# rapidsai/cugraph-gnn

Hardware: AMD Instinct MI355X
Metric: sampled-edges/sec (sample+renumber+feature-gather+SAGEConv fwd), ogbn-products-like fan-out [25, 10] (higher is better)
Workload: dtype int64 ids (int32 timed as a variant) + f32 features (SAGE lin_l/lin_r product: bf16x3-split MFMA, f32 accumulate); 1 GPU; ogbn-products-like RMAT: V=2449029, E=118462496 directed (CSR row_ptr i64 / col i64 replicated per GPU), feat fp32 [V,100], batch 1024/GPU, fan-out [25, 10], 2-layer SAGEConv(mean) 100-256-47 fwd, step = 8 call groups of 188 mini-batches; parallelism=dp1 (seeds sharded, no data-path collective)

## Files before the change

cugraph-gnn_amd/csrc/wg_rng.hpp:

```cpp
#pragma once
#include <hip/hip_runtime.h>

#include <cstdint>

namespace wgamd {

struct PcgJump {
  uint64_t a;
  uint64_t s;
};

struct PcgJumpTables {
  PcgJump t[4][256];
  constexpr PcgJumpTables() : t{}
  {
    uint64_t base_a = 6364136223846793005ULL, base_s = 1;
    for (int k = 0; k < 4; k++) {
      t[k][0].a = 1;
      t[k][0].s = 0;
      for (int c = 1; c < 256; c++) {
        t[k][c].a = t[k][c - 1].a * base_a;
        t[k][c].s = t[k][c - 1].s * base_a + base_s;
      }
      for (int d = 0; d < 8; d++) {
        uint64_t na = base_a * base_a, ns = base_s * base_a + base_s;
        base_a = na;
        base_s = ns;
      }
    }
  }
};

__device__ __constant__ const PcgJumpTables g_pcg_jump{};

struct Pcg32 {
  uint64_t state;
  uint64_t inc;

  static constexpr uint64_t kMult = 6364136223846793005ULL;

  __host__ __device__ __forceinline__ uint32_t next_u32()
  {
    uint64_t old = state;
    state        = old * kMult + inc;
    uint32_t x   = (uint32_t)(((old >> 18u) ^ old) >> 27u);
    uint32_t rot = (uint32_t)(old >> 59u);
    return (x >> rot) | (x << ((0u - rot) & 31u));
  }

  __host__ __device__ __forceinline__ void skipahead(uint64_t delta)
  {
    uint64_t acc_mult = 1u, acc_plus = 0u, cur_mult = kMult, cur_plus = inc;
    while (delta) {
      if (delta & 1u) {
        acc_mult *= cur_mult;
        acc_plus = acc_plus * cur_mult + cur_plus;
      }
      cur_plus = (cur_mult + 1u) * cur_plus;
      cur_mult *= cur_mult;
      delta >>= 1u;
    }
    state = acc_mult * state + acc_plus;
  }

  __host__ __device__ __forceinline__ Pcg32(uint64_t seed, uint64_t subsequence)
  {
    state = 0u;
    inc   = (subsequence << 1u) | 1u;
    (void)next_u32();
    state += seed;
    (void)next_u32();
    skipahead(subsequence);
  }

  __device__ __forceinline__ void jump_table(uint32_t n)
  {
    PcgJump j = g_pcg_jump.t[0][n & 255u];
#pragma unroll
    for (int k = 1; k < 4; k++) {
      const uint32_t c = (n >> (8 * k)) & 255u;
      if (c) {
        const PcgJump m = g_pcg_jump.t[k][c];
        j.s             = j.s * m.a + m.s;
        j.a             = j.a * m.a;
      }
    }
    state = j.a * state + inc * j.s;
  }

  struct table_tag {};
  __device__ __forceinline__ Pcg32(uint64_t seed, uint32_t subsequence, table_tag, uint32_t extra_draws = 0)
  {
    inc   = ((uint64_t)subsequence << 1u) | 1u;
    state = (inc + seed) * kMult + inc;
    jump_table(subsequence + extra_draws);
  }

  __host__ __device__ __forceinline__ int32_t next_i31() { return (int32_t)(next_u32() & 0x7fffffffu); }
  __host__ __device__ __forceinline__ uint64_t next_u64()
  {
    uint64_t lo = next_u32();
    uint64_t hi = next_u32();
    return lo | (hi << 32u);
  }
  __host__ __device__ __forceinline__ int64_t next_i63() { return (int64_t)(next_u64() & 0x7fffffffffffffffULL); }
  __host__ __device__ __forceinline__ float next_f32() { return (float)(next_u32() >> 8u) / 16777216.0f; }
};

}
```

cugraph-gnn_amd/csrc/wg_sample.hip:

```cpp
#include <algorithm>
#include <cmath>

#include "wg_common.hpp"
#include "wg_rng.hpp"

namespace wgamd {
namespace {

template <typename T>
struct dtype_of;
template <>
struct dtype_of<int32_t> {
  static constexpr wholememory_dtype_t value = WHOLEMEMORY_DT_INT;
};
template <>
struct dtype_of<int64_t> {
  static constexpr wholememory_dtype_t value = WHOLEMEMORY_DT_INT64;
};

__host__ __device__ constexpr int ref_block_threads(int M)
{
  int f = (M - 1) / 32;
  return f < 3 ? 32 : f < 6 ? 64 : f < 12 ? 128 : 256;
}
// ... 48 lines not shown
        deg = (M > 0 && deg > M) ? M : deg;
      }
      cnt[i] = deg;
      if (big_deg) big_deg[i] = 0;
    }
    return;
  }
  int i = blockIdx.x * blockDim.x + threadIdx.x;
  int cls          = -1;
  int deg          = 0;
  if (i < n_.host) {
    if (i >= n_live) {
      if (i < (n_live / kScanTile + 1) * kScanTile) {
        cnt[i] = 0;
        if (big_deg) big_deg[i] = 0;
      }
    } else {
      int64_t nid         = (int64_t)seeds[i];
      const int64_t first = row_ptr[nid];
      deg                 = (int)(row_ptr[nid + 1] - first);
      cnt[i]              = (M > 0 && deg > M) ? M : deg;
      if (row_start) {
        row_start[i] = first;
        row_deg[i]   = deg;
      }
      if (big_deg) big_deg[i] = 0;
      if (lists != nullptr && M > 0 && deg > M) {
        cls = deg <= 16 ? 0 : deg <= 32 ? 1 : deg <= 64 ? 2 : deg <= 128 ? 3 : deg <= 256 ? 4 : deg <= 512 ? 5
              : deg <= kWaveRowCapDecl ? 6 : deg <= kHugeRow ? 7 : 8;
        if (cls >= 7 && deg > scratch_threshold) atomicMax(lists + 10, deg);
      }
    }
  }
  if (lists == nullptr) return;
  __shared__ int blk_cnt[kWeightedLists], blk_base[kWeightedLists];
  if (threadIdx.x < kWeightedLists) blk_cnt[threadIdx.x] = 0;
  __syncthreads();
  const int lane = threadIdx.x & 63;
  int my_rank    = 0;
#pragma unroll
  for (int c = 0; c < kWeightedLists; c++) {
    const uint64_t m = __ballot(cls == c);
    if (m == 0ull) continue;
    const int leader = __ffsll((long long)m) - 1;
    int base         = 0;
    if (lane == leader) base = atomicAdd(&blk_cnt[c], __popcll(m));
    base = __shfl(base, leader, 64);
    if (cls == c) my_rank = base + __popcll(m & ((1ull << lane) - 1ull));
  }
  __syncthreads();
  if (threadIdx.x < kWeightedLists && blk_cnt[threadIdx.x] > 0) blk_base[threadIdx.x] = atomicAdd(lists + threadIdx.x, blk_cnt[threadIdx.x]);
  __syncthreads();
  if (cls >= 0) lists[kWeightedListHead + (int64_t)cls * list_cap + blk_base[cls] + my_rank] = i;
}

template <typename ColT>
__device__ __forceinline__ ColT col_at(const ColT* __restrict__ col, int64_t at)
{
  return col ? col[at] : (ColT)0;
}

constexpr int kWalkGrid = 256 * 16;

template <typename ColT>
__device__ __forceinline__ void emit(ColT* dst, int* src_lid, int64_t* edge_gid, int64_t out, ColT v,
                                     int seed_index, int64_t gid)
{
  if (dst) dst[out] = v;
  if (src_lid) src_lid[out] = seed_index;
  if (edge_gid) edge_gid[out] = gid;
}

struct loc_rec {
  int64_t start;
  int i;
  int deg;
  int base;
  int i_local;
  int batch;
  int pad;
};
static_assert(sizeof(loc_rec) == 32, "one 32-byte sector per record");
constexpr int kLocBuckets = 4096;
constexpr int kLocBlocks  = 128;
constexpr int kLocThreads = 1024;

template <typename SeedT>
__global__ void __launch_bounds__(kLocThreads)
locality_hist_kernel(const SeedT* __restrict__ seeds, dev_count n_, int shift, int* __restrict__ hist )
{
  __shared__ int h[kLocBuckets];
  const int n = n_.get(), per = (n + kLocBlocks - 1) / kLocBlocks;
  const int lo = min(n, (int)blockIdx.x * per), hi = min(n, lo + per);
  for (int k = threadIdx.x; k < kLocBuckets; k += kLocThreads) h[k] = 0;
  __syncthreads();
  for (int i = lo + threadIdx.x; i < hi; i += kLocThreads)
    atomicAdd(&h[min((int)((uint64_t)seeds[i] >> shift), kLocBuckets - 1)], 1);
  __syncthreads();
  for (int k = threadIdx.x; k < kLocBuckets; k += kLocThreads) hist[(int64_t)blockIdx.x * kLocBuckets + k] = h[k];
}

template <typename SeedT>
__global__ void __launch_bounds__(kLocThreads)
locality_scatter_kernel(const SeedT* __restrict__ seeds, dev_count n_, int shift, const int* __restrict__ hist,
                        const int64_t* __restrict__ row_start, const int* __restrict__ row_deg, const int* __restrict__ offsets,
                        rng_plan rng, loc_rec* __restrict__ recs)
{
  __shared__ int cursor[kLocBuckets];
  __shared__ int wave_tot[kLocThreads / 64];
  static_assert(kLocBuckets == 4 * kLocThreads, "thread t owns buckets 4 t .. 4 t + 3");
  const int n = n_.get(), per = (n + kLocBlocks - 1) / kLocBlocks;
  const int lo = min(n, (int)blockIdx.x * per), hi = min(n, lo + per);
  int tot[4] = {0, 0, 0, 0}, before[4] = {0, 0, 0, 0};
  const int4* h4 = reinterpret_cast<const int4*>(hist);
  for (int b = 0; b < kLocBlocks; b++) {
    const int4 v = h4[(int64_t)b * (kLocBuckets / 4) + threadIdx.x];
    tot[0] += v.x; tot[1] += v.y; tot[2] += v.z; tot[3] += v.w;
    if (b < (int)blockIdx.x) { before[0] += v.x; before[1] += v.y; before[2] += v.z; before[3] += v.w; }
  }
  const int sum = tot[0] + tot[1] + tot[2] + tot[3];
  int inc = sum;
  const int lane = threadIdx.x & 63, wave = threadIdx.x >> 6;
#pragma unroll
  for (int d = 1; d < 64; d <<= 1) {
    const int up = __shfl_up(inc, d, 64);
    if (lane >= d) inc += up;
  }
  if (lane == 63) wave_tot[wave] = inc;
  __syncthreads();
  int run = inc - sum;
  for (int w = 0; w < wave; w++) run += wave_tot[w];
#pragma unroll
  for (int k = 0; k < 4; k++) {
    cursor[4 * threadIdx.x + k] = run + before[k];
    run += tot[k];
  }
  __syncthreads();
  for (int i = lo + threadIdx.x; i < hi; i += kLocThreads) {
    const int j = atomicAdd(&cursor[min((int)((uint64_t)seeds[i] >> shift), kLocBuckets - 1)], 1);
    loc_rec r;
    r.start = row_start[i];
    r.i     = i;
    r.deg   = row_deg[i];
    r.base  = offsets[i];
    r.i_local = i;
    r.batch   = 0;
    if (rng.target_batch) {
      r.batch   = rng.target_batch[i];
      r.i_local = i - rng.target_seg[r.batch];
    }
    r.pad   = 0;
    recs[j] = r;
  }
}

template <typename SeedT, typename ColT, int LANES>
__global__ void __launch_bounds__(256) sample_uniform_halfwave_kernel(const int64_t* __restrict__ row_ptr,
                                                                      const ColT* __restrict__ col,
                                                                      const SeedT* __restrict__ seeds,
                                                                      dev_count n_,
                                                                      int M,
                                                                      rng_plan rng,
                                                                      const int* __restrict__ offsets,
                                                                      ColT* __restrict__ dst,
                                                                      int* __restrict__ src_lid,
                                                                      int64_t* __restrict__ edge_gid,
                                                                      const int64_t* __restrict__ row_start,
                                                                      const int* __restrict__ row_deg,
                                                                      const loc_rec* __restrict__ recs = nullptr)
{
  const int n    = n_.get();
  const int lane = threadIdx.x & 63;
  const int hl   = lane & (LANES - 1);
  const int hb   = lane & ~(LANES - 1);
  int i          = (int)(((int64_t)blockIdx.x * blockDim.x + threadIdx.x) / LANES);
  loc_rec rec{};
  if (recs) {
    constexpr int kGroups = 256 / LANES;
    const int per_x = ((n + 7) / 8 + kGroups - 1) / kGroups * kGroups;
    const int k     = (int)(blockIdx.x >> 3) * kGroups + (int)threadIdx.x / LANES;
    const int j     = (int)(blockIdx.x & 7) * per_x + k;
    i               = n;
    if (k < per_x && j < n) {
      rec = recs[j];
      i   = rec.i;
    }
  }
  int32_t r_draw = 0;
  if (i < n && hl < M) {
    uint64_t random_seed;
    int i_local;
    if (recs) {
      i_local     = rec.i_local;
      random_seed = rng.seeds_dev ? rng.seeds_dev[rec.batch] : rng.seed;
    } else
      rng.resolve(i, random_seed, i_local);
    if (i_local < (1 << 26)) {
      Pcg32 g(random_seed, (uint32_t)(i_local * 32 + hl), Pcg32::table_tag{});
      r_draw = g.next_i31();
    } else {
      Pcg32 g(random_seed, stream_id(i_local, 32, hl));
      r_draw = g.next_i31();
    }
  }
  int64_t start = 0;
  int N = 0, base = 0;
  if (i < n && recs) {
    start = rec.start;
    N     = rec.deg;
    base  = rec.base;
  } else if (i < n) {
    if (row_start) {
      start = row_start[i];
      N     = row_deg[i];
    } else {
      int64_t nid = (int64_t)seeds[i];
      start       = row_ptr[nid];
      N           = (int)(row_ptr[nid + 1] - start);
    }
    base = offsets[i];
  }
  const bool pick = N > M;
  if (__ballot(pick) == 0ull) {
    if (hl < N) emit<ColT>(dst, src_lid, edge_gid, (int64_t)base + hl, col_at<ColT>(col, start + hl), i, start + hl);
    return;
  }
  int r = 0;
  if (pick && hl < M) r = r_draw % (N - hl);
  const int tail = N - hl - 1;
  int p1 = -1, p2 = -1;
  for (int s = 0; s + 1 < M; s++) {
    const int rs    = __shfl(r, hb | s, 64);
    const bool prev = s < hl;
    p1 = (prev && rs == r) ? s : p1;
    p2 = (prev && rs == tail) ? s : p2;
  }
  int root = p2 >= 0 ? p2 : hl;
#pragma unroll
  for (int round = 0; round < (LANES == 32 ? 5 : 4); round++) root = __shfl(root, hb | root, 64);
  const int val = N - root - 1;
  const int vp1 = __shfl(val, hb | (p1 & (LANES - 1)), 64);
  const int a   = p1 >= 0 ? vp1 : r;
  if (pick) {
    if (hl < M) emit<ColT>(dst, src_lid, edge_gid, (int64_t)base + hl, col_at<ColT>(col, start + a), i, start + a);
  } else if (hl < N) {
    emit<ColT>(dst, src_lid, edge_gid, (int64_t)base + hl, col_at<ColT>(col, start + hl), i, start + hl);
  }
}

template <typename SeedT, typename ColT, int GW, int K, bool EXACT>
__global__ void __launch_bounds__(256)
sample_uniform_multi_kernel(const ColT* __restrict__ col, dev_count n_, int M_rt, rng_plan rng, const int* __restrict__ offsets,
                            ColT* __restrict__ dst, int* __restrict__ src_lid, int64_t* __restrict__ edge_gid,
                            const int64_t* __restrict__ row_start, const int* __restrict__ row_deg,
                            const loc_rec* __restrict__ recs)
{
  constexpr int kGPW    = 64 / GW;
  constexpr int kGroups = 4 * kGPW;
  constexpr int kRounds = GW <= 2 ? 1 : GW <= 4 ? 2 : GW <= 8 ? 3 : GW <= 16 ? 4 : 5;
  const int M    = EXACT ? GW : M_rt;
  const int n    = n_.get();
  const int lane = threadIdx.x & 63;
  const int grp  = lane / GW;
  const int hl   = lane - grp * GW;
  const int hb   = grp * GW;
  const bool live_group = grp < kGPW;
  const int wg_group    = (int)(threadIdx.x >> 6) * kGPW + grp;
  const int per_x = ((n + 7) / 8 + kGroups * K - 1) / (kGroups * K) * (kGroups * K);
  const int64_t n_chunks = recs ? (int64_t)(per_x / (kGroups * K)) * 8 : ((int64_t)n + kGroups * K - 1) / (kGroups * K);
  for (int64_t chunk = blockIdx.x; chunk < n_chunks; chunk += gridDim.x) {
  int i[K], N[K], base[K], i_local[K], batch[K];
  int64_t start[K];
  if (recs) {
    const int k0    = ((int)(chunk >> 3) * kGroups + wg_group) * K;
#pragma unroll
    for (int k = 0; k < K; k++) {
      const int j = (int)(chunk & 7) * per_x + k0 + k;
      i[k] = n, N[k] = 0, base[k] = 0, start[k] = 0, i_local[k] = 0, batch[k] = 0;
      if (live_group && k0 + k < per_x && j < n) {
        const loc_rec r = recs[j];
        i[k] = r.i, N[k] = r.deg, base[k] = r.base, start[k] = r.start, i_local[k] = r.i_local, batch[k] = r.batch;
      }
    }
  } else {
    const int64_t g = chunk * kGroups + wg_group;
#pragma unroll
    for (int k = 0; k < K; k++) {
      i[k] = live_group ? (int)min(g * K + k, (int64_t)n) : n;
      N[k] = 0, base[k] = 0, start[k] = 0, i_local[k] = i[k], batch[k] = 0;
      if (i[k] < n) {
        start[k] = row_start[i[k]];
        N[k]     = row_deg[i[k]];
        base[k]  = offsets[i[k]];
        if (rng.target_batch) batch[k] = rng.target_batch[i[k]];
      }
    }
    if (rng.target_batch) {
#pragma unroll
      for (int k = 0; k < K; k++)
        if (i[k] < n) i_local[k] = i[k] - rng.target_seg[batch[k]];
    }
  }
  int32_t r_draw[K];
#pragma unroll
  for (int k = 0; k < K; k++) {
    r_draw[k] = 0;
    if (i[k] < n && hl < M) {
      const uint64_t random_seed = rng.seeds_dev ? rng.seeds_dev[rng.target_batch ? batch[k] : 0] : rng.seed;
      if (i_local[k] < (1 << 26)) {
        Pcg32 g(random_seed, (uint32_t)(i_local[k] * 32 + hl), Pcg32::table_tag{});
        r_draw[k] = g.next_i31();
      } else {
        Pcg32 g(random_seed, stream_id(i_local[k], 32, hl));
        r_draw[k] = g.next_i31();
      }
    }
  }
  int a[K];
#pragma unroll
  for (int k = 0; k < K; k++) {
    const bool pick = N[k] > M;
    a[k]            = hl;
    if (__ballot(pick) != 0ull) {
      int r = 0;
      if (pick && hl < M) r = r_draw[k] % (N[k] - hl);
      const int tail = N[k] - hl - 1;
      int p1 = -1, p2 = -1;
      auto step = [&](int s) {
        const int rs    = __shfl(r, hb + s, 64);
        const bool prev = s < hl;
        p1 = (prev && rs == r) ? s : p1;
        p2 = (prev && rs == tail) ? s : p2;
      };
      if constexpr (EXACT) {
#pragma unroll
        for (int s = 0; s + 1 < GW; s++) step(s);
      } else {
        for (int s = 0; s + 1 < M; s++) step(s);
      }
      int root = p2 >= 0 ? p2 : hl;
#pragma unroll
      for (int round = 0; round < kRounds; round++) root = __shfl(root, hb + root, 64);
      const int val = N[k] - root - 1;
      const int vp1 = __shfl(val, hb + max(p1, 0), 64);
      if (pick) a[k] = p1 >= 0 ? vp1 : r;
    }
  }
  ColT v[K];
  bool on[K];
#pragma unroll
  for (int k = 0; k < K; k++) {
    on[k] = live_group && hl < (N[k] > M ? M : N[k]);
    v[k]  = on[k] ? col_at<ColT>(col, start[k] + a[k]) : (ColT)0;
  }
#pragma unroll
  for (int k = 0; k < K; k++)
    if (on[k]) emit<ColT>(dst, src_lid, edge_gid, (int64_t)base[k] + hl, v[k], i[k], start[k] + a[k]);
  }
}

constexpr int kHashSlots = 4096;

__device__ __forceinline__ int lds_hash_find(const int* keys, int pos)
{
  uint32_t h = ((uint32_t)pos * 2654435761u) & (kHashSlots - 1);
  while (true) {
    int k = keys[h];
    if (k == pos || k == -1) return (int)h;
    h = (h + 1) & (kHashSlots - 1);
  }
}

template <typename SeedT, typename ColT>
__global__ void __launch_bounds__(256) sample_uniform_block_kernel(const int64_t* __restrict__ row_ptr,
                                                                   const ColT* __restrict__ col,
                                                                   const SeedT* __restrict__ seeds,
                                                                   dev_count n_,
                                                                   int M,
                                                                   int B,
                                                                   int items,
                                                                   rng_plan rng,
                                                                   const int* __restrict__ offsets,
                                                                   ColT* __restrict__ dst,
                                                                   int* __restrict__ src_lid,
                                                                   int64_t* __restrict__ edge_gid)
{
  __shared__ int r[1024];
  __shared__ int a[1024];
  __shared__ int hkeys[kHashSlots];
  __shared__ int hvals[kHashSlots];
  const int i = blockIdx.x;
  if (i >= n_.get()) return;
  const int64_t nid   = (int64_t)seeds[i];
  const int64_t start = row_ptr[nid];
  const int N         = (int)(row_ptr[nid + 1] - start);
  if (N <= 0) return;
  const int base = offsets[i];
  if (N <= M) {
    for (int j = threadIdx.x; j < N; j += blockDim.x)
      emit<ColT>(dst, src_lid, edge_gid, (int64_t)base + j, col_at<ColT>(col, start + j), i, start + j);
    return;
  }
  for (int h = threadIdx.x; h < kHashSlots; h += blockDim.x) hkeys[h] = -1;
  if ((int)threadIdx.x < B) {
    uint64_t random_seed;
    int i_local;
    rng.resolve(i, random_seed, i_local);
    Pcg32 g(random_seed, stream_id(i_local, B, threadIdx.x));
    for (int k = 0; k < items; k++) {
      int id = k * B + threadIdx.x;
      int v  = g.next_i31();
      if (id < M) r[id] = v % (N - id);
    }
  }
  __syncthreads();
  if (threadIdx.x == 0) {
    for (int t = 0; t < M; t++) {
      const int rt = r[t], tail = N - t - 1;
      int s1     = lds_hash_find(hkeys, rt);
      int q_rt   = hkeys[s1] == rt ? hvals[s1] : rt;
      int s2     = lds_hash_find(hkeys, tail);
      int q_tail = hkeys[s2] == tail ? hvals[s2] : tail;
      a[t]       = q_rt;
      hkeys[s1]  = rt;
      hvals[s1]  = q_tail;
    }
  }
  __syncthreads();
  for (int t = threadIdx.x; t < M; t += blockDim.x)
    emit<ColT>(dst, src_lid, edge_gid, (int64_t)base + t, col_at<ColT>(col, start + a[t]), i, start + a[t]);
}

template <typename SeedT, typename ColT>
__global__ void __launch_bounds__(64) sample_uniform_reservoir_kernel(const int64_t* __restrict__ row_ptr,
                                                                      const ColT* __restrict__ col,
                                                                      const SeedT* __restrict__ seeds,
                                                                      dev_count n_,
                                                                      int M,
                                                                      rng_plan rng,
                                                                      const int* __restrict__ offsets,
                                                                      ColT* __restrict__ dst,
                                                                      int* __restrict__ src_lid,
                                                                      int64_t* __restrict__ edge_gid)
{
  const int i = blockIdx.x;
  if (i >= n_.get()) return;
  const int64_t nid   = (int64_t)seeds[i];
  const int64_t start = row_ptr[nid];
  const int N         = (int)(row_ptr[nid + 1] - start);
  if (N <= 0) return;
  const int64_t base = offsets[i];
  if (N <= M) {
    for (int j = threadIdx.x; j < N; j += blockDim.x)
      emit<ColT>(dst, src_lid, edge_gid, base + j, col_at<ColT>(col, start + j), i, start + j);
    return;
  }
  for (int s = threadIdx.x; s < M; s += blockDim.x) dst[base + s] = (ColT)s;
  __syncthreads();
  if (threadIdx.x < 32) {
    uint64_t random_seed;
    int i_local;
    rng.resolve(i, random_seed, i_local);
    Pcg32 g(random_seed, stream_id(i_local, 32, threadIdx.x));
    for (int idx = M + threadIdx.x; idx < N; idx += 32) {
      int rn = g.next_i31() % (idx + 1);
      if (rn < M) {
        if constexpr (sizeof(ColT) == 8)
          atomicMax(reinterpret_cast<long long*>(dst + base + rn), (long long)idx);
        else
          atomicMax(reinterpret_cast<int*>(dst + base + rn), idx);
      }
    }
  }
  __syncthreads();
  for (int s = threadIdx.x; s < M; s += blockDim.x) {
    int sel = (int)__hip_atomic_load(dst + base + s, __ATOMIC_RELAXED, __HIP_MEMORY_SCOPE_AGENT);
    emit<ColT>(dst, src_lid, edge_gid, base + s, col_at<ColT>(col, start + sel), i, start + sel);
  }
}

__device__ __forceinline__ float ares_key(float w, Pcg32& g, bool* redrawn = nullptr)
{
  float u = g.next_f32();
  u       = (float)(-(0.5 + 0.5 * (double)u));
  uint64_t x;
  int zero_draws = -1;
  do {
    x = g.next_u64();
    zero_draws++;
  } while (!x);
  if (redrawn != nullptr && zero_draws > 0) *redrawn = true;
  int one_bit = __clzll((long long)x) + zero_draws * 64;
  u *= exp2f((float)(-one_bit));
#ifdef WG_TUNE_CHEAP_KEY
  return u * 1.442695f * __builtin_amdgcn_rcpf(w);
#endif
  return (log1pf(u) / logf(2.0f)) * (1.0f / w);
}

constexpr int kWaveRowCap = 1024;
static_assert(kWaveRowCap == kWaveRowCapDecl, "keep the two in step");

__device__ __forceinline__ uint32_t key_bits(float k)
{
  uint32_t b = __float_as_uint(k);
  return (b & 0x80000000u) ? ~b : (b | 0x80000000u);
}

constexpr int kLdsKeys = kWeightedLdsKeys;

template <typename SeedT, typename ColT, typename WeightT, int B, int T>
__global__ void __launch_bounds__(T) sample_weighted_kernel(const int64_t* __restrict__ row_ptr,
                                                            const ColT* __restrict__ col,
                                                            const WeightT* __restrict__ weight,
                                                            const SeedT* __restrict__ seeds,
                                                            dev_count n_,
                                                            int M,
                                                            rng_plan rng,
                                                            const int* __restrict__ offsets,
                                                            uint32_t* __restrict__ slab,
                                                            int64_t slab_len,
                                                            ColT* __restrict__ dst,
                                                            int* __restrict__ src_lid,
                                                            int64_t* __restrict__ edge_gid,
                                                            int* __restrict__ lists ,
                                                            int list_cap,
                                                            int redo = 0 )
{
  static_assert(T % B == 0 && T % 64 == 0, "threads must be a multiple of the stream layout and of the wave");
  __shared__ uint32_t lds_keys[kLdsKeys];
  __shared__ int hist[256];
  __shared__ int sh_digit, sh_need, sh_redo;
  __shared__ int wave_cnt[2][T / 64];
  __shared__ int sh_li;
  const int n_live  = n_.get();
  const int n_huge  = lists && !redo ? lists[8] : 0;
  const int count   = lists ? (redo ? lists[kWeightedRedoCount] : n_huge + lists[7]) : n_live;
  uint32_t* gkeys   = slab + (int64_t)blockIdx.x * slab_len;
  int li            = blockIdx.x;
  while (true) {
  __syncthreads();
  if (lists) {
    if (threadIdx.x == 0) sh_li = atomicAdd(lists + (redo ? kWeightedRedoHead : 9), 1);
    __syncthreads();
    li = sh_li;
  }
  if (li >= count) break;
  const int i = lists ? (redo ? lists[kWeightedListHead + (int64_t)kWeightedRedoList * list_cap + li]
                         : li < n_huge ? lists[kWeightedListHead + 8 * (int64_t)list_cap + li]
                                       : lists[kWeightedListHead + 7 * (int64_t)list_cap + (li - n_huge)])
                      : li;
  if (!lists) li += gridDim.x;
  if (i >= n_live) continue;
  uint64_t random_seed;
  int i_rng;
  rng.resolve(i, random_seed, i_rng);
  const int64_t nid   = (int64_t)seeds[i];
  const int64_t start = row_ptr[nid];
  const int N         = (int)(row_ptr[nid + 1] - start);
  if (N <= 0) continue;
  const int64_t base = offsets[i];
  if (M <= 0 || N <= M) {
    for (int j = threadIdx.x; j < N; j += T)
      emit<ColT>(dst, src_lid, edge_gid, base + j, col_at<ColT>(col, start + j), i, start + j);
    continue;
  }
  const bool in_lds = N <= kLdsKeys;
  auto put = [&](int id, uint32_t k) { if (in_lds) lds_keys[id] = k; else gkeys[id] = k; };
  auto get = [&](int id) -> uint32_t {
    return in_lds ? lds_keys[id] : __hip_atomic_load(gkeys + id, __ATOMIC_RELAXED, __HIP_MEMORY_SCOPE_AGENT);
  };
  if (threadIdx.x == 0) sh_redo = 0;
  __syncthreads();
  {
    constexpr int hop = T / B;
    const int lane = threadIdx.x % B, part = threadIdx.x / B;
    const int L     = lane < N ? (N - lane + B - 1) / B : 0;
    const int share = (L + hop - 1) / hop;
    const int m0 = part * share, m1 = min(L, m0 + share);
    bool redrawn = false;
    if (m0 < m1) {
      const int64_t sid = (int64_t)i_rng * B + lane;
      Pcg32 g = (sid < (1ll << 31)) ? Pcg32(random_seed, (uint32_t)sid, Pcg32::table_tag{}, 3u * (uint32_t)m0)
                                    : Pcg32(random_seed, stream_id(i_rng, B, lane));
      if (sid >= (1ll << 31)) g.skipahead(3u * (uint64_t)m0);
      for (int m = m0; m < m1; m++) {
        const int id = lane + m * B;
        put(id, key_bits(ares_key((float)weight[start + id], g, &redrawn)));
      }
    }
    if (redrawn) sh_redo = 1;
  }
  __syncthreads();
  if (T > B && sh_redo) {
    if (threadIdx.x < B) {
      Pcg32 g = stream_generator(random_seed, i_rng, B, threadIdx.x);
      for (int id = threadIdx.x; id < N; id += B) put(id, key_bits(ares_key((float)weight[start + id], g)));
    }
    __syncthreads();
  }
  uint32_t prefix = 0, prefix_mask = 0;
  int need = M;
  for (int shift = 24; shift >= 0; shift -= 8) {
    for (int h = threadIdx.x; h < 256; h += T) hist[h] = 0;
    __syncthreads();
    for (int id = threadIdx.x; id < N; id += T) {
      uint32_t k = get(id);
      if ((k & prefix_mask) == prefix) atomicAdd(&hist[(k >> shift) & 255], 1);
    }
    __syncthreads();
    if (threadIdx.x < 64) {
      const int l  = threadIdx.x;
      const int h0 = hist[4 * l], h1 = hist[4 * l + 1], h2 = hist[4 * l + 2], h3 = hist[4 * l + 3];
// ... 1252 lines not shown
```

cugraph-gnn_amd/csrc/wg_unique.hip:

```cpp
#include "wg_common.hpp"
#include "wgamd_ext.h"

namespace wgamd {
namespace {

template <typename IdT>
__global__ void __launch_bounds__(256) unique_mark_kernel(const IdT* __restrict__ ids, int64_t n, int64_t bound, uint8_t* __restrict__ flags,
                                                          int* __restrict__ bad, const int* __restrict__ n_live)
{
  if (n_live) n = min(n, (int64_t)*n_live);
  const int64_t T = (int64_t)gridDim.x * blockDim.x;
  for (int64_t i = (int64_t)blockIdx.x * blockDim.x + threadIdx.x; i < n; i += 4 * T) {
    int64_t id[4];
    uint8_t f[4];
#pragma unroll
    for (int k = 0; k < 4; k++) id[k] = i + k * T < n ? (int64_t)ids[i + k * T] : -1;
#pragma unroll
    for (int k = 0; k < 4; k++) {
      if (id[k] >= bound) {
        *bad  = 1;
        id[k] = -1;
      }
      f[k] = id[k] >= 0 ? flags[id[k]] : 1;
    }
#pragma unroll
    for (int k = 0; k < 4; k++)
      if (f[k] == 0) flags[id[k]] = 1;
  }
}

__global__ void __launch_bounds__(256) unique_pack_kernel(const uint8_t* __restrict__ flags, int64_t n_words, uint2* __restrict__ rank,
                                                          int* __restrict__ cnt, int64_t cnt_padded)
{
  const int64_t w = (int64_t)blockIdx.x * blockDim.x + threadIdx.x;
  if (w < n_words) {
    const uint4* p = reinterpret_cast<const uint4*>(flags + w * 32);
    const uint4 a = p[0], b = p[1];
    const uint32_t v[8] = {a.x, a.y, a.z, a.w, b.x, b.y, b.z, b.w};
    uint32_t word = 0;
#pragma unroll
    for (int k = 0; k < 8; k++) {
      const uint32_t x = v[k];
      word |= ((x & 1u) | ((x >> 7) & 2u) | ((x >> 14) & 4u) | ((x >> 21) & 8u)) << (4 * k);
    }
    rank[w].x = word;
    cnt[w]    = __popc(word);
  } else if (w < cnt_padded) {
    cnt[w] = 0;
  }
}

__global__ void __launch_bounds__(256) unique_compact_kernel(uint2* __restrict__ rank, const int* __restrict__ prefix, int64_t n_words,
                                                             int64_t* __restrict__ distinct, int* __restrict__ n_distinct)
{
  const int64_t w = (int64_t)blockIdx.x * blockDim.x + threadIdx.x;
  if (w == 0 && n_distinct) *n_distinct = prefix[n_words];
  if (w >= n_words) return;
  uint32_t word = rank[w].x;
  int at        = prefix[w];
  rank[w].y     = (uint32_t)at;
  while (word) {
    const int k    = __ffs(word) - 1;
    distinct[at++] = w * 32 + k;
    word &= word - 1;
  }
}

template <typename IdT>
__global__ void __launch_bounds__(256) unique_inverse_kernel(const IdT* __restrict__ ids, int64_t n, int64_t bound, const uint2* __restrict__ rank,
                                                             int* __restrict__ inverse,
                                                             const int* __restrict__ n_live)
{
  if (n_live) n = min(n, (int64_t)*n_live);
  const int64_t T = (int64_t)gridDim.x * blockDim.x;
  for (int64_t i = (int64_t)blockIdx.x * blockDim.x + threadIdx.x; i < n; i += 4 * T) {
    int64_t id[4];
    uint2 r[4];
#pragma unroll
    for (int k = 0; k < 4; k++) id[k] = i + k * T < n ? (int64_t)ids[i + k * T] : -1;
#pragma unroll
    for (int k = 0; k < 4; k++) {
      const bool ok = id[k] >= 0 && id[k] < bound;
      r[k]          = ok ? rank[id[k] >> 5] : make_uint2(0u, 0xffffffffu);
    }
#pragma unroll
    for (int k = 0; k < 4; k++)
      if (i + k * T < n) inverse[i + k * T] = (int)r[k].y + __popc(r[k].x & ((1u << (id[k] & 31)) - 1u));
  }
}

struct unique_plan {
  size_t flags, bits, cnt, tmp, bad, total;
  int64_t n_words, cnt_padded;
};
unique_plan plan_unique(int64_t bound)
{
  unique_plan p{};
  size_t at = 0;
  auto add  = [&](size_t bytes) {
    const size_t o = at;
    at += (bytes + 255) / 256 * 256;
    return o;
  };
  p.n_words    = (bound + 31) / 32;
  p.cnt_padded = (p.n_words + kScanTile) / kScanTile * kScanTile;
  p.flags = add((size_t)p.n_words * 32);
  p.bits  = add(sizeof(uint2) * (size_t)p.n_words);
  p.cnt   = add(sizeof(int) * (size_t)(p.cnt_padded + 1));
  p.tmp   = add(sizeof(int) * (size_t)scan_tmp_ints(p.n_words));
  p.bad   = add(sizeof(int));
  p.total = at;
  return p;
}

}
}

extern "C" {

size_t wgamd_unique_bounded_workspace_bytes(int64_t id_bound)
{
  if (id_bound <= 0 || id_bound >= ((int64_t)1 << 31) - 4096) return 0;
  return wgamd::plan_unique(id_bound).total;
}

wholememory_error_code_t wgamd_unique_bounded(const void* ids, wholememory_dtype_t id_dtype, int64_t n, int64_t id_bound,
                                              int64_t* distinct, int* inverse, int* n_distinct_dev, int* out_of_bound_dev,
                                              void* workspace, size_t workspace_bytes, void* stream)
{
  return wgamd_unique_bounded_live(ids, id_dtype, n, nullptr, id_bound, distinct, inverse, n_distinct_dev, out_of_bound_dev,
                                   workspace, workspace_bytes, stream);
}

wholememory_error_code_t wgamd_unique_bounded_live(const void* ids, wholememory_dtype_t id_dtype, int64_t n, const int* n_live_dev,
                                                   int64_t id_bound, int64_t* distinct, int* inverse, int* n_distinct_dev,
                                                   int* out_of_bound_dev, void* workspace, size_t workspace_bytes, void* stream)
{
  using namespace wgamd;
  return guarded("wgamd_unique_bounded", [&] {
    WG_REQUIRE_INPUT(id_dtype == WHOLEMEMORY_DT_INT || id_dtype == WHOLEMEMORY_DT_INT64, "id dtype must be INT|INT64");
    WG_REQUIRE_INPUT(n >= 0 && n < ((int64_t)1 << 31), "bad id count");
    WG_REQUIRE_INPUT(id_bound > 0 && id_bound < ((int64_t)1 << 31) - 4096, "id_bound must be in (0, 2^31)");
    WG_REQUIRE_INPUT(n_distinct_dev && workspace && (n == 0 || (ids && distinct && inverse)), "null pointer");
    const unique_plan p = plan_unique(id_bound);
    WG_REQUIRE_INPUT(workspace_bytes >= p.total, "workspace too small: need %zu bytes", p.total);
    WG_REQUIRE_INPUT((reinterpret_cast<uintptr_t>(workspace) & 255) == 0, "workspace must be 256-byte aligned");
    hipStream_t st = static_cast<hipStream_t>(stream);
    char* base     = static_cast<char*>(workspace);
    uint8_t* flags = reinterpret_cast<uint8_t*>(base + p.flags);
    uint2* rank    = reinterpret_cast<uint2*>(base + p.bits);
    int* cnt       = reinterpret_cast<int*>(base + p.cnt);
    int* tmp       = reinterpret_cast<int*>(base + p.tmp);
    int* bad       = reinterpret_cast<int*>(base + p.bad);
    WG_HIP_CHECK(hipMemsetAsync(flags, 0, (size_t)p.n_words * 32, st));
    WG_HIP_CHECK(hipMemsetAsync(bad, 0, sizeof(int), st));
    if (n > 0) {
      const int grid = (int)std::min<int64_t>(ceil_div(n, 256), 256 * 32);
      if (id_dtype == WHOLEMEMORY_DT_INT) unique_mark_kernel<int32_t><<<grid, 256, 0, st>>>(static_cast<const int32_t*>(ids), n, id_bound, flags, bad, n_live_dev);
      else unique_mark_kernel<int64_t><<<grid, 256, 0, st>>>(static_cast<const int64_t*>(ids), n, id_bound, flags, bad, n_live_dev);
      WG_HIP_CHECK(hipGetLastError());
    }
    unique_pack_kernel<<<(int)ceil_div(p.cnt_padded, 256), 256, 0, st>>>(flags, p.n_words, rank, cnt, p.cnt_padded);
    exclusive_scan_i32(cnt, cnt, p.n_words, tmp, st);
    unique_compact_kernel<<<(int)ceil_div(p.n_words, 256), 256, 0, st>>>(rank, cnt, p.n_words, distinct, n_distinct_dev);
    WG_HIP_CHECK(hipGetLastError());
    if (n > 0) {
      const int grid = (int)std::min<int64_t>(ceil_div(n, 256), 256 * 32);
      if (id_dtype == WHOLEMEMORY_DT_INT) unique_inverse_kernel<int32_t><<<grid, 256, 0, st>>>(static_cast<const int32_t*>(ids), n, id_bound, rank, inverse, n_live_dev);
      else unique_inverse_kernel<int64_t><<<grid, 256, 0, st>>>(static_cast<const int64_t*>(ids), n, id_bound, rank, inverse, n_live_dev);
      WG_HIP_CHECK(hipGetLastError());
    }
    if (out_of_bound_dev) WG_HIP_CHECK(hipMemcpyAsync(out_of_bound_dev, bad, sizeof(int), hipMemcpyDeviceToDevice, st));
  });
}

}
```

Measured before the change: 5.377 billion sampled-edges/s.

## Replicate unique flag planes, fuse scan into pack/compact, and reuse PCG jump maps

The unique path now spreads mark writes over up to eight replicated flag planes when a plane fits in about 3 MB, so concurrent blocks contend less on the same flag bytes. The pack kernel ORs the planes together and writes per-tile popcount sums. A compact kernel does the block scan with a carry, replacing the separate global scan, memsets and D2D copy with fewer launches. Separately, the sampler reuses the previous PCG jump map when consecutive rows are adjacent, composing one table step instead of four lookups. The costs are extra plane memory and clear bandwidth, plus a serial per-tile carry loop in compact.

```diff
diff --git a/cugraph-gnn_amd/csrc/wg_rng.hpp b/cugraph-gnn_amd/csrc/wg_rng.hpp
--- a/cugraph-gnn_amd/csrc/wg_rng.hpp
+++ b/cugraph-gnn_amd/csrc/wg_rng.hpp
@@ -73,27 +73,32 @@
     skipahead(subsequence);
   }
 
-  __device__ __forceinline__ void jump_table(uint32_t n)
+  __host__ __device__ __forceinline__ static PcgJump compose(const PcgJump& n, const PcgJump& m) { return PcgJump{n.a * m.a, n.s * m.a + m.s}; }
+
+  __device__ __forceinline__ static PcgJump jump_map(uint32_t n)
   {
     PcgJump j = g_pcg_jump.t[0][n & 255u];
 #pragma unroll
     for (int k = 1; k < 4; k++) {
       const uint32_t c = (n >> (8 * k)) & 255u;
-      if (c) {
-        const PcgJump m = g_pcg_jump.t[k][c];
-        j.s             = j.s * m.a + m.s;
-        j.a             = j.a * m.a;
-      }
+      if (c) j = compose(j, g_pcg_jump.t[k][c]);
     }
-    state = j.a * state + inc * j.s;
+    return j;
+  }
+
+  __host__ __device__ __forceinline__ void jump(const PcgJump& j) { state = j.a * state + inc * j.s; }
+
+  __device__ __forceinline__ Pcg32(uint64_t seed, uint32_t subsequence, const PcgJump& j)
+  {
+    inc   = ((uint64_t)subsequence << 1u) | 1u;
+    state = (inc + seed) * kMult + inc;
+    jump(j);
   }
 
   struct table_tag {};
   __device__ __forceinline__ Pcg32(uint64_t seed, uint32_t subsequence, table_tag, uint32_t extra_draws = 0)
+      : Pcg32(seed, subsequence, jump_map(subsequence + extra_draws))
   {
-    inc   = ((uint64_t)subsequence << 1u) | 1u;
-    state = (inc + seed) * kMult + inc;
-    jump_table(subsequence + extra_draws);
   }
 
   __host__ __device__ __forceinline__ int32_t next_i31() { return (int32_t)(next_u32() & 0x7fffffffu); }
diff --git a/cugraph-gnn_amd/csrc/wg_sample.hip b/cugraph-gnn_amd/csrc/wg_sample.hip
--- a/cugraph-gnn_amd/csrc/wg_sample.hip
+++ b/cugraph-gnn_amd/csrc/wg_sample.hip
@@ -374,13 +374,19 @@
     }
   }
   int32_t r_draw[K];
+  PcgJump jmap{};
+  int jmap_of = -2;
 #pragma unroll
   for (int k = 0; k < K; k++) {
     r_draw[k] = 0;
     if (i[k] < n && hl < M) {
       const uint64_t random_seed = rng.seeds_dev ? rng.seeds_dev[rng.target_batch ? batch[k] : 0] : rng.seed;
       if (i_local[k] < (1 << 26)) {
-        Pcg32 g(random_seed, (uint32_t)(i_local[k] * 32 + hl), Pcg32::table_tag{});
+        const uint32_t sid = (uint32_t)(i_local[k] * 32 + hl);
+        if (i_local[k] == jmap_of + 1) jmap = Pcg32::compose(jmap, g_pcg_jump.t[0][32]);
+        else jmap = Pcg32::jump_map(sid);
+        jmap_of = i_local[k];
+        Pcg32 g(random_seed, sid, jmap);
         r_draw[k] = g.next_i31();
       } else {
         Pcg32 g(random_seed, stream_id(i_local[k], 32, hl));
diff --git a/cugraph-gnn_amd/csrc/wg_unique.hip b/cugraph-gnn_amd/csrc/wg_unique.hip
--- a/cugraph-gnn_amd/csrc/wg_unique.hip
+++ b/cugraph-gnn_amd/csrc/wg_unique.hip
@@ -4,11 +4,24 @@
 namespace wgamd {
 namespace {
 
+constexpr int kMaxPlanes = 8;
+constexpr int64_t kPlaneL2Bytes = (int64_t)3 << 20;
+constexpr int kTileWords = 256;
+
+__global__ void __launch_bounds__(256) unique_clear_kernel(uint4* __restrict__ planes, int64_t n16, int* __restrict__ bad)
+{
+  const int64_t T = (int64_t)gridDim.x * blockDim.x;
+  for (int64_t i = (int64_t)blockIdx.x * blockDim.x + threadIdx.x; i < n16; i += T) planes[i] = make_uint4(0u, 0u, 0u, 0u);
+  if (blockIdx.x == 0 && threadIdx.x == 0) *bad = 0;
+}
+
 template <typename IdT>
-__global__ void __launch_bounds__(256) unique_mark_kernel(const IdT* __restrict__ ids, int64_t n, int64_t bound, uint8_t* __restrict__ flags,
-                                                          int* __restrict__ bad, const int* __restrict__ n_live)
+__global__ void __launch_bounds__(256) unique_mark_kernel(const IdT* __restrict__ ids, int64_t n, int64_t bound, uint8_t* __restrict__ planes,
+                                                          int64_t plane_bytes, int plane_mask, int* __restrict__ bad,
+                                                          const int* __restrict__ n_live)
 {
   if (n_live) n = min(n, (int64_t)*n_live);
+  uint8_t* __restrict__ flags = planes + (int64_t)(blockIdx.x & plane_mask) * plane_bytes;
   const int64_t T = (int64_t)gridDim.x * blockDim.x;
   for (int64_t i = (int64_t)blockIdx.x * blockDim.x + threadIdx.x; i < n; i += 4 * T) {
     int64_t id[4];
@@ -29,40 +42,101 @@
   }
 }
 
-__global__ void __launch_bounds__(256) unique_pack_kernel(const uint8_t* __restrict__ flags, int64_t n_words, uint2* __restrict__ rank,
-                                                          int* __restrict__ cnt, int64_t cnt_padded)
-{
-  const int64_t w = (int64_t)blockIdx.x * blockDim.x + threadIdx.x;
+__device__ __forceinline__ int block_sum_256(int v)
+{
+  __shared__ int wave_sums[4];
+#pragma unroll
+  for (int d = 32; d >= 1; d >>= 1) v += __shfl_xor(v, d, 64);
+  if ((threadIdx.x & 63) == 0) wave_sums[threadIdx.x >> 6] = v;
+  __syncthreads();
+  const int total = wave_sums[0] + wave_sums[1] + wave_sums[2] + wave_sums[3];
+  __syncthreads();
+  return total;
+}
+
+__device__ __forceinline__ int block_exclusive_scan_256(int v, int* total)
+{
+  __shared__ int wave_sums[4];
+  const int lane = threadIdx.x & 63, wave = threadIdx.x >> 6;
+  int inc = v;
+#pragma unroll
+  for (int d = 1; d < 64; d <<= 1) {
+    const int up = __shfl_up(inc, d, 64);
+    if (lane >= d) inc += up;
+  }
+  if (lane == 63) wave_sums[wave] = inc;
+  __syncthreads();
+  int before = 0, tot = 0;
+#pragma unroll
+  for (int w = 0; w < 4; w++) {
+    const int s = wave_sums[w];
+    before += w < wave ? s : 0;
+    tot += s;
+  }
+  __syncthreads();
+  *total = tot;
+  return before + inc - v;
+}
+
+__global__ void __launch_bounds__(kTileWords) unique_pack_kernel(const uint8_t* __restrict__ planes, int64_t plane_bytes, int n_planes,
+                                                                 int64_t n_words, uint2* __restrict__ rank, int* __restrict__ tile_sums)
+{
+  const int64_t w = (int64_t)blockIdx.x * kTileWords + threadIdx.x;
+  uint32_t word   = 0;
   if (w < n_words) {
-    const uint4* p = reinterpret_cast<const uint4*>(flags + w * 32);
-    const uint4 a = p[0], b = p[1];
+    uint4 a = make_uint4(0u, 0u, 0u, 0u), b = a;
+#pragma unroll
+    for (int p = 0; p < kMaxPlanes; p++) {
+      if (p < n_planes) {
+        const uint4* q = reinterpret_cast<const uint4*>(planes + p * plane_bytes + w * 32);
+        const uint4 x = q[0], y = q[1];
+        a.x |= x.x, a.y |= x.y, a.z |= x.z, a.w |= x.w;
+        b.x |= y.x, b.y |= y.y, b.z |= y.z, b.w |= y.w;
+      }
+    }
     const uint32_t v[8] = {a.x, a.y, a.z, a.w, b.x, b.y, b.z, b.w};
-    uint32_t word = 0;
 #pragma unroll
     for (int k = 0; k < 8; k++) {
       const uint32_t x = v[k];
       word |= ((x & 1u) | ((x >> 7) & 2u) | ((x >> 14) & 4u) | ((x >> 21) & 8u)) << (4 * k);
     }
     rank[w].x = word;
-    cnt[w]    = __popc(word);
-  } else if (w < cnt_padded) {
-    cnt[w] = 0;
-  }
-}
-
-__global__ void __launch_bounds__(256) unique_compact_kernel(uint2* __restrict__ rank, const int* __restrict__ prefix, int64_t n_words,
-                                                             int64_t* __restrict__ distinct, int* __restrict__ n_distinct)
-{
-  const int64_t w = (int64_t)blockIdx.x * blockDim.x + threadIdx.x;
-  if (w == 0 && n_distinct) *n_distinct = prefix[n_words];
-  if (w >= n_words) return;
-  uint32_t word = rank[w].x;
-  int at        = prefix[w];
-  rank[w].y     = (uint32_t)at;
-  while (word) {
-    const int k    = __ffs(word) - 1;
-    distinct[at++] = w * 32 + k;
-    word &= word - 1;
+  }
+  const int total = block_sum_256(__popc(word));
+  if (threadIdx.x == 0) tile_sums[blockIdx.x] = total;
+}
+
+__global__ void __launch_bounds__(kTileWords) unique_compact_kernel(uint2* __restrict__ rank, const int* __restrict__ tile_sums, int64_t n_tiles,
+                                                                    int64_t n_words, int64_t* __restrict__ distinct, int* __restrict__ n_distinct,
+                                                                    const int* __restrict__ bad, int* __restrict__ out_of_bound)
+{
+  const int64_t per   = (n_tiles + gridDim.x - 1) / gridDim.x;
+  const int64_t first = (int64_t)blockIdx.x * per, last = min(n_tiles, first + per);
+  if (blockIdx.x == 0) {
+    int part = 0;
+    for (int64_t t = threadIdx.x; t < n_tiles; t += kTileWords) part += tile_sums[t];
+    const int total = block_sum_256(part);
+    if (threadIdx.x == 0) {
+      *n_distinct = total;
+      if (out_of_bound) *out_of_bound = *bad;
+    }
+  }
+  if (first >= last) return;
+  int part = 0;
+  for (int64_t t = threadIdx.x; t < first; t += kTileWords) part += tile_sums[t];
+  int carry = block_sum_256(part);
+  for (int64_t tile = first; tile < last; tile++) {
+    const int64_t w = tile * kTileWords + threadIdx.x;
+    uint32_t word   = w < n_words ? rank[w].x : 0u;
+    int total;
+    int at = block_exclusive_scan_256(__popc(word), &total) + carry;
+    if (w < n_words) rank[w].y = (uint32_t)at;
+    while (word) {
+      const int k    = __ffs(word) - 1;
+      distinct[at++] = w * 32 + k;
+      word &= word - 1;
+    }
+    carry += total;
   }
 }
 
@@ -90,8 +164,9 @@
 }
 
 struct unique_plan {
-  size_t flags, bits, cnt, tmp, bad, total;
-  int64_t n_words, cnt_padded;
+  size_t planes, bits, sums, bad, total;
+  int64_t n_words, n_tiles, plane_bytes;
+  int n_planes;
 };
 unique_plan plan_unique(int64_t bound)
 {
@@ -102,14 +177,15 @@
     at += (bytes + 255) / 256 * 256;
     return o;
   };
-  p.n_words    = (bound + 31) / 32;
-  p.cnt_padded = (p.n_words + kScanTile) / kScanTile * kScanTile;
-  p.flags = add((size_t)p.n_words * 32);
-  p.bits  = add(sizeof(uint2) * (size_t)p.n_words);
-  p.cnt   = add(sizeof(int) * (size_t)(p.cnt_padded + 1));
-  p.tmp   = add(sizeof(int) * (size_t)scan_tmp_ints(p.n_words));
-  p.bad   = add(sizeof(int));
-  p.total = at;
+  p.n_words     = (bound + 31) / 32;
+  p.n_tiles     = (p.n_words + kTileWords - 1) / kTileWords;
+  p.plane_bytes = (p.n_words * 32 + 255) / 256 * 256;
+  p.n_planes    = p.plane_bytes <= kPlaneL2Bytes ? kMaxPlanes : 1;
+  p.planes      = add((size_t)p.n_planes * (size_t)p.plane_bytes);
+  p.bits        = add(sizeof(uint2) * (size_t)p.n_words);
+  p.sums        = add(sizeof(int) * (size_t)p.n_tiles);
+  p.bad         = add(sizeof(int));
+  p.total       = at;
   return p;
 }
 
@@ -145,32 +221,29 @@
     const unique_plan p = plan_unique(id_bound);
     WG_REQUIRE_INPUT(workspace_bytes >= p.total, "workspace too small: need %zu bytes", p.total);
     WG_REQUIRE_INPUT((reinterpret_cast<uintptr_t>(workspace) & 255) == 0, "workspace must be 256-byte aligned");
-    hipStream_t st = static_cast<hipStream_t>(stream);
-    char* base     = static_cast<char*>(workspace);
-    uint8_t* flags = reinterpret_cast<uint8_t*>(base + p.flags);
-    uint2* rank    = reinterpret_cast<uint2*>(base + p.bits);
-    int* cnt       = reinterpret_cast<int*>(base + p.cnt);
-    int* tmp       = reinterpret_cast<int*>(base + p.tmp);
-    int* bad       = reinterpret_cast<int*>(base + p.bad);
-    WG_HIP_CHECK(hipMemsetAsync(flags, 0, (size_t)p.n_words * 32, st));
-    WG_HIP_CHECK(hipMemsetAsync(bad, 0, sizeof(int), st));
+    hipStream_t st  = static_cast<hipStream_t>(stream);
+    char* base      = static_cast<char*>(workspace);
+    uint8_t* planes = reinterpret_cast<uint8_t*>(base + p.planes);
+    uint2* rank     = reinterpret_cast<uint2*>(base + p.bits);
+    int* sums       = reinterpret_cast<int*>(base + p.sums);
+    int* bad        = reinterpret_cast<int*>(base + p.bad);
+    const int64_t n16 = (int64_t)p.n_planes * p.plane_bytes / 16;
+    unique_clear_kernel<<<(int)std::min<int64_t>(ceil_div(n16, 4 * 256), 4096), 256, 0, st>>>(reinterpret_cast<uint4*>(planes), n16, bad);
+    const int grid = (int)std::min<int64_t>(ceil_div(n, 256), 256 * 32);
     if (n > 0) {
-      const int grid = (int)std::min<int64_t>(ceil_div(n, 256), 256 * 32);
-      if (id_dtype == WHOLEMEMORY_DT_INT) unique_mark_kernel<int32_t><<<grid, 256, 0, st>>>(static_cast<const int32_t*>(ids), n, id_bound, flags, bad, n_live_dev);
-      else unique_mark_kernel<int64_t><<<grid, 256, 0, st>>>(static_cast<const int64_t*>(ids), n, id_bound, flags, bad, n_live_dev);
-      WG_HIP_CHECK(hipGetLastError());
-    }
-    unique_pack_kernel<<<(int)ceil_div(p.cnt_padded, 256), 256, 0, st>>>(flags, p.n_words, rank, cnt, p.cnt_padded);
-    exclusive_scan_i32(cnt, cnt, p.n_words, tmp, st);
-    unique_compact_kernel<<<(int)ceil_div(p.n_words, 256), 256, 0, st>>>(rank, cnt, p.n_words, distinct, n_distinct_dev);
-    WG_HIP_CHECK(hipGetLastError());
+      if (id_dtype == WHOLEMEMORY_DT_INT)
+        unique_mark_kernel<int32_t><<<grid, 256, 0, st>>>(static_cast<const int32_t*>(ids), n, id_bound, planes, p.plane_bytes, p.n_planes - 1, bad, n_live_dev);
+      else
+        unique_mark_kernel<int64_t><<<grid, 256, 0, st>>>(static_cast<const int64_t*>(ids), n, id_bound, planes, p.plane_bytes, p.n_planes - 1, bad, n_live_dev);
+    }
+    unique_pack_kernel<<<(int)p.n_tiles, kTileWords, 0, st>>>(planes, p.plane_bytes, p.n_planes, p.n_words, rank, sums);
+    unique_compact_kernel<<<(int)std::min<int64_t>(p.n_tiles, 1024), kTileWords, 0, st>>>(rank, sums, p.n_tiles, p.n_words, distinct, n_distinct_dev,
+                                                                                          bad, out_of_bound_dev);
     if (n > 0) {
-      const int grid = (int)std::min<int64_t>(ceil_div(n, 256), 256 * 32);
       if (id_dtype == WHOLEMEMORY_DT_INT) unique_inverse_kernel<int32_t><<<grid, 256, 0, st>>>(static_cast<const int32_t*>(ids), n, id_bound, rank, inverse, n_live_dev);
       else unique_inverse_kernel<int64_t><<<grid, 256, 0, st>>>(static_cast<const int64_t*>(ids), n, id_bound, rank, inverse, n_live_dev);
-      WG_HIP_CHECK(hipGetLastError());
-    }
-    if (out_of_bound_dev) WG_HIP_CHECK(hipMemcpyAsync(out_of_bound_dev, bad, sizeof(int), hipMemcpyDeviceToDevice, st));
+    }
+    WG_HIP_CHECK(hipGetLastError());
   });
 }
 
```

Measured after the change: 5.439 billion sampled-edges/s, median of 6. About the same (+1.1%).
